# xbpeng/DeepMimic

Measured on NVIDIA H100. Metric: env-steps/sec (30 Hz policy steps; humanoid3d_spinkick, 4096 envs/GPU), higher is better.
Workload: dtype f32

## Files before the change

deepmimic_b200/capi.py:

```python
import ctypes as C
import os

import numpy as np

_REPO = os.path.dirname(os.path.dirname(os.path.abspath(__file__)))
_LIB_PATH = os.environ.get("DM_LIB", os.path.join(_REPO, "deepmimic_b200", "libdeepmimic_b200.so"))
_lib = None


class DmDims(C.Structure):
    _fields_ = [(n, C.c_int) for n in ("num_envs", "num_joints", "pose_dim", "num_dofs", "state_size", "goal_size", "action_size", "snapshot_size",
                                        "updates_per_action", "num_update_substeps")] + [("motion_duration", C.c_double), ("amp_obs_size", C.c_int)]


_fp = C.POINTER(C.c_float)


class DmMlpGatedWeights(C.Structure):
    _fields_ = ([(n, C.c_int) for n in ("in_dim", "goal_dim", "h0", "h1", "out_dim", "gate_common", "gate_hidden")]
                + [(n, _fp) for n in ("w0", "b0", "w1", "b1", "w2", "b2", "gc_w", "gc_b")]
                + [(n, _fp * 2) for n in ("gh_w", "gh_b", "gs_w", "gs_b", "gb_w", "gb_b")]
                + [(n, _fp) for n in ("s_mean", "s_std", "g_mean", "g_std", "a_mean", "a_std")] + [("s_clip", C.c_float), ("g_clip", C.c_float)])


# ... 6 lines not shown
                + [(n, C.c_void_p) for n in ("norm_actions", "old_logp", "adv", "logstd", "bound_min", "bound_max")]
                + [("ratio_clip", C.c_float), ("ratio", C.c_void_p), ("norm_targets", C.c_void_p)]
                + [(n, C.c_float) for n in ("stepsize", "momentum", "weight_decay")] + [("stats", C.c_void_p)])


class DmLearnDiscBatch(C.Structure):
    _fields_ = ([(n, C.c_void_p) for n in ("agent", "expert", "agent_idx", "expert_idx")] + [("rows", C.c_int), ("in_mean", C.c_void_p),
                ("in_istd", C.c_void_p), ("in_clip", C.c_float)]
                + [(n, C.c_float) for n in ("stepsize", "momentum", "weight_decay", "logit_reg_weight", "grad_penalty_weight")] + [("stats", C.c_void_p)])


class DmLearnGatedNet(C.Structure):
    _fields_ = [(n, C.c_void_p * 10) for n in ("w", "b", "acc_w", "acc_b")]


class DmLearnGatedBatch(C.Structure):
    _anonymous_ = ("batch",)
    _fields_ = [("batch", DmLearnBatch), ("goals", C.c_void_p), ("g_mean", C.c_void_p), ("g_istd", C.c_void_p), ("g_clip", C.c_float)]


DM_STATE_OFFSET, DM_STATE_SCALE, DM_ACTION_OFFSET, DM_ACTION_SCALE, DM_ACTION_BOUND_MIN, DM_ACTION_BOUND_MAX, DM_STATE_NORM_GROUPS = range(7)

EXPORTS = ["dm_create", "dm_load_host", "dm_plan_launch", "dm_get_model_info", "dm_get_link_table", "dm_destroy", "dm_last_error", "dm_get_dims", "dm_get_static", "dm_get_scene_name", "dm_stream", "dm_sync", "dm_set_mode", "dm_set_sample_count", "dm_get_time_limits", "dm_reset", "dm_set_action",
           "dm_update", "dm_record_state", "dm_record_goal", "dm_goal_host", "dm_reset_clips", "dm_record_amp_obs_expert_clips", "dm_get_clip_table", "dm_get_task_state", "dm_set_task_state", "dm_get_task_params", "dm_calc_reward", "dm_calc_reward_imitate", "dm_record_amp_obs_agent", "dm_record_amp_obs_expert", "dm_amp_obs_host", "dm_sample_amp_obs_expert", "dm_expert_sample_count", "dm_observe", "dm_get_flags", "dm_step_host", "dm_step_host_reset", "dm_set_time_limits", "dm_exchange_create", "dm_exchange_connect", "dm_exchange_publish", "dm_exchange_acquire", "dm_exchange_release", "dm_exchange_status", "dm_exchange_destroy", "dm_set_timing", "dm_step_host_timing", "dm_get_snapshot",
           "dm_set_snapshot", "dm_get_counters", "dm_get_section_profile", "dm_mlp_create", "dm_mlp_forward", "dm_mlp_create_gated", "dm_mlp_forward_gated",
           "dm_mlp_forward_style_reward", "dm_mlp_launches", "dm_mlp_destroy", "dm_td_lambda_returns", "dm_mlp_set_weights_device", "dm_learn_create",
           "dm_mlp_set_normalizers_device", "dm_learn_set_weights", "dm_learn_step", "dm_learn_disc_step", "dm_learn_destroy",
           "dm_learn_create_gated", "dm_learn_set_gated_weights", "dm_learn_gated_step", "dm_mlp_set_gated_weights_device", "dm_mlp_set_gated_normalizers_device"]


def lib():
    global _lib
    if _lib is None:
        if not os.path.exists(_LIB_PATH):
            raise RuntimeError("deepmimic_b200: %s is missing -- run `python -c 'import __graft_entry__ as g; g.build()'`. "
                               "There is no CPU fallback." % _LIB_PATH)
        L = C.CDLL(_LIB_PATH)
        vp, dp, fp, ip = C.c_void_p, C.POINTER(C.c_double), C.c_void_p, C.c_void_p
        L.dm_create.restype = vp
        L.dm_create.argtypes = [C.c_char_p, C.c_int, C.POINTER(C.c_char_p), C.c_int, C.c_int, C.c_uint64, C.c_uint64]
        L.dm_destroy.argtypes = [vp]
        L.dm_load_host.restype = vp
        L.dm_load_host.argtypes = [C.c_char_p, C.c_int, C.POINTER(C.c_char_p)]
        L.dm_get_model_info.argtypes = [vp, C.c_int, C.POINTER(C.c_int)]
        L.dm_plan_launch.argtypes = [vp, C.c_int, C.c_int, C.c_int, C.POINTER(C.c_int)]
        L.dm_get_link_table.argtypes = [vp, dp]
        L.dm_last_error.restype = C.c_char_p
        L.dm_get_dims.argtypes = [vp, C.POINTER(DmDims)]
        L.dm_get_static.argtypes = [vp, C.c_int, dp]
        L.dm_get_scene_name.argtypes = [vp, C.c_char_p, C.c_int]
        L.dm_stream.restype = vp
        L.dm_stream.argtypes = [vp]
        L.dm_sync.argtypes = [vp]
        L.dm_set_mode.argtypes = [vp, C.c_int]
        L.dm_set_sample_count.argtypes = [vp, C.c_longlong]
        L.dm_get_time_limits.argtypes = [vp, dp]
        L.dm_reset.argtypes = [vp, C.c_int, dp, dp, dp]
        L.dm_set_action.argtypes = [vp, fp]
        L.dm_update.argtypes = [vp, C.c_double, C.c_int]
        L.dm_record_state.argtypes = [vp, fp]
        L.dm_record_goal.argtypes = [vp, fp]
        L.dm_calc_reward.argtypes = [vp, fp]
        L.dm_calc_reward_imitate.argtypes = [vp, fp]
        L.dm_goal_host.argtypes = [vp, fp]
        L.dm_reset_clips.argtypes = [vp, C.c_int, C.POINTER(C.c_int), dp, dp, dp]
        L.dm_record_amp_obs_expert_clips.argtypes = [vp, C.POINTER(C.c_int), dp, fp]
        L.dm_get_clip_table.argtypes = [vp, C.POINTER(C.c_int), dp, dp]
        L.dm_get_task_state.argtypes = [vp, C.c_int, dp]
        L.dm_set_task_state.argtypes = [vp, C.c_int, dp]
        L.dm_get_task_params.argtypes = [vp, dp, C.POINTER(C.c_uint64)]
        L.dm_record_amp_obs_agent.argtypes = [vp, fp]
        L.dm_record_amp_obs_expert.argtypes = [vp, dp, fp]
        L.dm_amp_obs_host.argtypes = [vp, C.c_int, dp, fp]
        L.dm_sample_amp_obs_expert.argtypes = [vp, C.c_int, vp, vp, vp]
        L.dm_expert_sample_count.argtypes = [vp, C.POINTER(C.c_uint64), C.POINTER(C.c_uint64)]
        L.dm_observe.argtypes = [vp, fp, fp]
        L.dm_get_flags.argtypes = [vp, ip]
        L.dm_step_host.argtypes = [vp, fp, C.c_double, C.c_int, fp, fp, ip]
        L.dm_step_host_reset.argtypes = [vp, fp, C.c_double, C.c_int, fp, fp, ip, C.c_int]
        L.dm_set_time_limits.argtypes = [vp, C.c_double, C.c_double]
        L.dm_exchange_create.argtypes = [vp, C.c_int, C.c_int, C.c_void_p]
        L.dm_exchange_connect.argtypes = [vp, C.c_void_p]
# ... 48 lines not shown


def _dptr(a):
    return a.ctypes.data_as(C.POINTER(C.c_double)) if a is not None else None


def _call(fn, *args, stream=None):
    if getattr(lib(), fn)(*args, C.c_void_p(stream) if stream else None) != 0:
        raise RuntimeError("%s: %s" % (fn, lib().dm_last_error().decode()))


def td_lambda_returns(rewards, values, end_values, done, terminate, discount, td_lambda, val_fail, val_succ, returns, advantages, stream=None):
    T, N = rewards.shape
    for name, x, dt in (("rewards", rewards, "float32"), ("values", values, "float32"), ("end_values", end_values, "float32"), ("returns", returns, "float32"),
                        ("advantages", advantages, "float32"), ("done", done, ("bool", "uint8")), ("terminate", terminate, "int32")):
        if tuple(x.shape) != (T, N) or not x.is_contiguous() or not x.is_cuda or str(x.dtype).replace("torch.", "") not in (dt if isinstance(dt, tuple) else (dt,)):
            raise ValueError("td_lambda_returns: %s must be a contiguous %s CUDA tensor [%d, %d]" % (name, dt, T, N))
    ptr = lambda t: C.c_void_p(t.data_ptr())
    _call("dm_td_lambda_returns", ptr(rewards), ptr(values), ptr(end_values), ptr(done), ptr(terminate), T, N, float(discount), float(td_lambda),
          float(val_fail), float(val_succ), ptr(returns), ptr(advantages), stream=stream)
    return returns, advantages


class BatchedCore:

    def __init__(self, args, num_envs, asset_root, device=0, seed=0, global_env_offset=0):
        L = lib()
        enc = [a.encode() for a in args]
        arr = (C.c_char_p * len(enc))(*enc)
        self.h = L.dm_create(asset_root.encode(), len(enc), arr, num_envs, device, seed, global_env_offset)
        if not self.h:
            raise RuntimeError("dm_create failed: %s" % L.dm_last_error().decode())
        self.h = C.c_void_p(self.h)
        d = DmDims()
        L.dm_get_dims(self.h, C.byref(d))
        self.dims = d
        self.num_envs = d.num_envs

    def _chk(self, rc):
        if rc != 0:
            raise RuntimeError("deepmimic_b200: %s" % lib().dm_last_error().decode())

    def close(self):
        if self.h:
            lib().dm_destroy(self.h)
            self.h = None
# ... 16 lines not shown
        return buf.value.decode()

    def reset(self, force_all=True, kin_time=None, max_time=None, rot_theta=None, clip=None):
        f = lambda a: None if a is None else np.ascontiguousarray(a, dtype=np.float64)
        kt, mt, th = f(kin_time), f(max_time), f(rot_theta)
        if clip is None:
            self._chk(lib().dm_reset(self.h, 1 if force_all else 0, _dptr(kt), _dptr(mt), _dptr(th)))
        else:
            c = np.ascontiguousarray(clip, dtype=np.int32)
            self._chk(lib().dm_reset_clips(self.h, 1 if force_all else 0, c.ctypes.data_as(C.POINTER(C.c_int)), _dptr(kt), _dptr(mt), _dptr(th)))

    def clip_table(self):
        n = C.c_int(0)
        lib().dm_get_clip_table(self.h, C.byref(n), None, None)
        dur, cdf = np.zeros(n.value), np.zeros(n.value)
        lib().dm_get_clip_table(self.h, C.byref(n), _dptr(dur), _dptr(cdf))
        return dur, cdf

    def set_action(self, actions):
        self._chk(lib().dm_set_action(self.h, C.c_void_p(actions.data_ptr())))

    def update(self, dt, n_updates=1):
        self._chk(lib().dm_update(self.h, dt, n_updates))

    def observe(self, state=None, reward=None):
        self._chk(lib().dm_observe(self.h, C.c_void_p(state.data_ptr()) if state is not None else None,
                                   C.c_void_p(reward.data_ptr()) if reward is not None else None))

    def reward_imitate(self, out):
        self._chk(lib().dm_calc_reward_imitate(self.h, C.c_void_p(out.data_ptr())))

    def record_goal(self, out):
        self._chk(lib().dm_record_goal(self.h, C.c_void_p(out.data_ptr())))

    def goal_host(self):
        out = np.zeros((self.num_envs, self.dims.goal_size), dtype=np.float32)
        self._chk(lib().dm_goal_host(self.h, C.c_void_p(out.ctypes.data)))
        return out

    def task_state(self, env):
        out = np.zeros(24, dtype=np.float64)
        self._chk(lib().dm_get_task_state(self.h, env, _dptr(out)))
        return out

    def set_task_state(self, env, block):
        b = np.ascontiguousarray(block, dtype=np.float64)
# ... 414 lines not shown
```

deepmimic_b200/csrc/capi.cu:

```cuda
#include <cuda_runtime.h>

#include <algorithm>
#include <map>
#include <mutex>
#include <cmath>
#include <cstddef>
#include <cstdio>
#include <cstdlib>
#include <numeric>
#include <cstring>
#include <ctime>
#include <utility>
#include <memory>
#include <string>
#include <vector>

#include "../../include/deepmimic_b200.h"
#include "host/assets.hpp"
#include "kernels/dm_model.cuh"

namespace dmk {
__global__ void dm_flags_kernel(DevState st, int32_t* out, int num_real_envs) {
    int e = blockIdx.x * blockDim.x + threadIdx.x;
    if (e >= num_real_envs) return;
// ... 43 lines not shown
        cudaError_t e_ = (call);                                                                              \
        if (e_ != cudaSuccess) { g_err = std::string(#call) + ": " + cudaGetErrorString(e_); return fail(); } \
    } while (0)

struct dm_handle {
    dmh::SceneAssets sa;
    dmk::DevModel hm;
    dmk::DevModel* d_model = nullptr;
    dmk::DevState st{};
    double* d_frame_times = nullptr;
    float* d_frames = nullptr;
    float* d_frame_vel = nullptr;
    double* d_inj[3] = {nullptr, nullptr, nullptr};
    int32_t* d_flags4 = nullptr;
    float *d_amp = nullptr, *p_amp = nullptr;
    float *d_goal = nullptr, *p_goal = nullptr;
    dmk::ClipTable ctab{};
    dmk::ClipTable* d_ctab = nullptr; int* d_clip_inj = nullptr;
    int total_frames = 0;
    float *d_act = nullptr, *d_obs = nullptr, *d_rew = nullptr;
    float *p_act = nullptr, *p_obs = nullptr, *p_rew = nullptr; int32_t* p_flags = nullptr;
    cudaStream_t stream = nullptr;
    int device = 0, num_envs = 0, padded_envs = 0, W = 32, tiles = 2, maxrows = 36, smem_bytes = 0, mode = 0;
    dmk::StepLayout lay{};
    uint64_t seed = 0, env_offset = 0;
    int64_t launches = 0;
    uint64_t amp_calls = 0;
    uint64_t expert_samples = 0;
    std::vector<double> st_off, st_scale, act_off, act_scale, act_min, act_max, st_groups;
    std::vector<std::pair<const void*, bool>> pin_cache;
    int x_rank = 0, x_world = 0;
    char* x_base = nullptr;
    char* x_peer[8] = {nullptr, nullptr, nullptr, nullptr, nullptr, nullptr, nullptr, nullptr};
    size_t x_data_off = 0, x_parity_bytes = 0;
    bool timing = false;
    cudaEvent_t tev[5] = {nullptr, nullptr, nullptr, nullptr, nullptr};
    double host_ms[3] = {0, 0, 0};
    std::vector<void*> dev_bufs, pinned_bufs;
};

namespace {

int fail() { std::fprintf(stderr, "[deepmimic_b200] %s\n", g_err.c_str()); return 1; }

using dmh::Quat; using dmh::V3;
inline void put3(float* o, const V3& v, double s = 1.0) { o[0] = static_cast<float>(s * v.x); o[1] = static_cast<float>(s * v.y); o[2] = static_cast<float>(s * v.z); }
// ... 202 lines not shown
}

bool task_scene(const dm_handle* h) { return h->hm.task_kind != dmk::kTaskNone; }
int goal_size(const dmk::DevModel& M) { return M.task_kind == dmk::kTaskNone ? 0 : (M.task_kind >= dmk::kTaskHeadingGetup ? 4 : 3); }
int tile_index(const dm_handle* h) { return h->W == 32 ? 1 : 0; }
int policy_grid(const dm_handle* h) { return h->padded_envs / (dmk::kPolicyBlock / h->W); }

int launched(dm_handle* h) {
    DM_CUDA(cudaGetLastError());
    h->launches++;
    return 0;
}

int launch_step(dm_handle* h, double dt, int n_updates) {
    const dmk::StepKernel kern = dmk::kStepKernels[tile_index(h)][task_scene(h)];
    static std::mutex mu;
    static std::map<std::pair<int, const void*>, int> configured;
    {
        std::lock_guard<std::mutex> lock(mu);
        int& have = configured[{h->device, reinterpret_cast<const void*>(kern)}];
        if (h->smem_bytes > have) {
            DM_CUDA(cudaFuncSetAttribute(kern, cudaFuncAttributeMaxDynamicSharedMemorySize, h->smem_bytes));
            DM_CUDA(cudaFuncSetAttribute(kern, cudaFuncAttributePreferredSharedMemoryCarveout, 100));
            have = h->smem_bytes;
        }
    }
    kern<<<h->padded_envs / h->tiles, h->tiles * h->W, h->smem_bytes, h->stream>>>(h->d_model, h->st, h->d_frame_times, h->d_frames, dt, n_updates,
                                                                                   h->sa.cfg.num_sim_substeps, h->lay);
    return launched(h);
}
int launch_observe_fan(dm_handle* h, const dmk::ObsFan& fan) {
    const dmk::ObserveKernel kern = dmk::kObserveKernels[tile_index(h)][task_scene(h)];
    const size_t smem = static_cast<size_t>(dmk::kPolicyBlock / h->W) * h->hm.state_size * sizeof(float);
    kern<<<policy_grid(h), dmk::kPolicyBlock, smem, h->stream>>>(h->d_model, h->st, h->d_frame_times, h->d_frames, h->d_frame_vel, fan, h->num_envs);
    return launched(h);
}
int launch_observe(dm_handle* h, float* d_state, float* d_reward) {
    dmk::ObsFan fan{};
    fan.n = 1; fan.obs[0] = d_state; fan.rew[0] = d_reward; fan.done[0] = nullptr;
    return launch_observe_fan(h, fan);
}
int launch_reset(dm_handle* h, int force, const double* kt, const double* mt, const double* th, const int* clip) {
    const dmk::ResetKernel kern = dmk::kResetKernels[tile_index(h)][task_scene(h)];
    kern<<<policy_grid(h), dmk::kPolicyBlock, 0, h->stream>>>(h->d_model, h->st, h->d_frame_times, h->d_frames, h->d_frame_vel, force, kt, mt, th, h->seed,
                                                              h->env_offset, h->mode, clip);
    return launched(h);
}
int launch_amp(dm_handle* h, float* d_out, int expert, const double* d_times, const int* d_clips) {
// ... 197 lines not shown
    h->ctab = dmk::ClipTable{};
    h->ctab.num_clips = static_cast<int>(h->sa.clips.size());
    for (size_t c = 0; c < h->sa.clips.size(); ++c) {
        const dmh::MotionClip& mc = h->sa.clips[c];
        dmk::ClipInfo& ci = h->ctab.info[c];
        ci.dur = mc.duration(); ci.frame_off = h->total_frames; ci.num_frames = mc.num_frames; ci.loop = mc.loop ? 1 : 0;
        const double* fb = mc.frame(0); const double* fe = mc.frame(mc.num_frames - 1);
        ci.cycle_delta[0] = static_cast<float>(fe[0] - fb[0]); ci.cycle_delta[1] = 0.f; ci.cycle_delta[2] = static_cast<float>(fe[2] - fb[2]);
        h->ctab.cdf[c] = h->sa.clip_cdf[c];
        ci.is_getup = std::find(h->sa.cfg.getup_motion_ids.begin(), h->sa.cfg.getup_motion_ids.end(), static_cast<int>(c)) != h->sa.cfg.getup_motion_ids.end() ? 1 : 0;
        h->total_frames += mc.num_frames;
    }
    const size_t TF = static_cast<size_t>(h->total_frames);
    DM_CUDA(cudaStreamCreateWithFlags(&h->stream, cudaStreamNonBlocking));
    if (alloc_buffer(h, &h->d_model, 1) || alloc_buffer(h, &h->st.sim, N * ss) || alloc_buffer(h, &h->st.time, N * dmk::kTimeDoubles, kZeroed) ||
        alloc_buffer(h, &h->st.flags, N * dmk::kFlagInts, kZeroed) || alloc_buffer(h, &h->st.manifold, N * M.nl * dmk::kManifoldFloats, kZeroed) ||
        alloc_buffer(h, &h->d_frame_times, TF) || alloc_buffer(h, &h->d_frames, TF * M.pose_dim) || alloc_buffer(h, &h->d_frame_vel, TF * M.pose_dim) ||
        alloc_buffer(h, &h->d_flags4, N * 4) || alloc_buffer(h, &h->d_amp, N * M.amp_obs_size) || alloc_buffer(h, &h->p_amp, N * M.amp_obs_size, kPinned) ||
        alloc_buffer(h, &h->st.hist, N * 2 * M.pose_dim, kZeroed) || alloc_buffer(h, &h->d_act, N * std::max(1, M.action_size)) ||
        alloc_buffer(h, &h->d_obs, N * M.state_size) || alloc_buffer(h, &h->d_rew, N) || alloc_buffer(h, &h->p_act, N * std::max(1, M.action_size), kPinned) ||
        alloc_buffer(h, &h->p_obs, N * M.state_size, kPinned) || alloc_buffer(h, &h->p_rew, N, kPinned) || alloc_buffer(h, &h->p_flags, N * 4, kPinned))
        return 1;
    for (auto& p : h->d_inj) if (alloc_buffer(h, &p, N)) return 1;
#ifdef DM_PROFILE
    if (alloc_buffer(h, &h->st.prof, static_cast<size_t>(h->padded_envs / h->tiles) * (h->tiles * h->W / 32) * dmk::kProfCounters, kZeroed)) return 1;
#endif
    h->st.num_envs = h->padded_envs; h->st.num_real = h->num_envs;
    if (task_scene(h)) {
        if (alloc_buffer(h, &h->st.task, N * dmk::kTaskDoubles, kZeroed) || alloc_buffer(h, &h->st.taskx, N * dmk::kTaskExtDoubles, kZeroed) ||
            alloc_buffer(h, &h->d_goal, N * 4) || alloc_buffer(h, &h->p_goal, N * 4, kPinned) || alloc_buffer(h, &h->st.clip, N, kZeroed) ||
            alloc_buffer(h, &h->d_clip_inj, N) || alloc_buffer(h, &h->d_ctab, 1))
            return 1;
        DM_CUDA(cudaMemcpy(h->d_ctab, &h->ctab, sizeof(dmk::ClipTable), cudaMemcpyHostToDevice));
    }
    h->st.ctab = h->d_ctab;
    std::vector<float> frames(TF * M.pose_dim), fvel(frames.size());
    std::vector<double> ftimes(TF);
    for (size_t c = 0; c < h->sa.clips.size(); ++c) {
        const dmh::MotionClip& mc = h->sa.clips[c];
        const std::vector<double> fv = build_frame_vel(h->sa.character, mc);
        const size_t off = static_cast<size_t>(h->ctab.info[c].frame_off);
        std::copy(mc.frame_times.begin(), mc.frame_times.end(), ftimes.begin() + off);
        for (size_t i = 0; i < mc.frames.size(); ++i) { frames[off * M.pose_dim + i] = static_cast<float>(mc.frames[i]); fvel[off * M.pose_dim + i] = static_cast<float>(fv[i]); }
    }
    DM_CUDA(cudaMemcpy(h->d_model, &h->hm, sizeof(dmk::DevModel), cudaMemcpyHostToDevice));
    DM_CUDA(cudaMemcpy(h->d_frame_times, ftimes.data(), sizeof(double) * TF, cudaMemcpyHostToDevice));
// ... 109 lines not shown
    for (int k = 0; k < 3; ++k) if (src[k] && stage_envs(h, src[k], h->d_inj[k])) return 1;
    if (h_clip && stage_envs(h, h_clip, h->d_clip_inj)) return 1;
    if (launch_reset(h, force_all, kt ? h->d_inj[0] : nullptr, mt ? h->d_inj[1] : nullptr, th ? h->d_inj[2] : nullptr, h_clip ? h->d_clip_inj : nullptr)) return 1;
    if (!task_scene(h)) return 0;
    dmk::dm_task_reset_kernel<<<(h->padded_envs + 127) / 128, 128, 0, h->stream>>>(h->d_model, h->st, h->padded_envs);
    return launched(h);
}
int dm_reset(dm_handle* h, int force_all, const double* kt, const double* mt, const double* th) { return dm_reset_clips(h, force_all, nullptr, kt, mt, th); }
int dm_get_clip_table(dm_handle* h, int* num_clips, double* h_dur, double* h_cdf) {
    const int n = static_cast<int>(h->sa.clips.size());
    if (num_clips) *num_clips = n;
    for (int c = 0; c < n; ++c) { if (h_dur) h_dur[c] = h->sa.clips[c].duration(); if (h_cdf) h_cdf[c] = h->sa.clip_cdf[c]; }
    return 0;
}
int dm_set_action(dm_handle* h, const float* d_actions) {
    DM_DEVICE(h);
    const int total = h->num_envs * h->hm.nl;
    dmk::dm_set_action_kernel<<<(total + 127) / 128, 128, 0, h->stream>>>(h->d_model, h->st, d_actions, h->num_envs);
    return launched(h);
}
int dm_update(dm_handle* h, double dt, int n_updates) {
    DM_DEVICE(h);
    return launch_step(h, dt, n_updates);
}
static int launch_task_observe(dm_handle* h, float* d_goal, float* d_reward) {
    dmk::dm_task_observe_kernel<<<(h->num_envs + 127) / 128, 128, 0, h->stream>>>(h->d_model, h->st, d_goal, d_reward, h->num_envs);
    return launched(h);
}
int dm_observe(dm_handle* h, float* d_state, float* d_reward) {
    DM_DEVICE(h);
    const bool task = task_scene(h);
    float* d_imitate_reward = task ? nullptr : d_reward;
    if ((d_state != nullptr || d_imitate_reward != nullptr) && launch_observe(h, d_state, d_imitate_reward)) return 1;
    if (task && d_reward != nullptr) return launch_task_observe(h, nullptr, d_reward);
    return 0;
}
int dm_record_state(dm_handle* h, float* d_out) { return dm_observe(h, d_out, nullptr); }
int dm_calc_reward_imitate(dm_handle* h, float* d_out) {
    DM_DEVICE(h);
    return launch_observe(h, nullptr, d_out);
}
int dm_record_goal(dm_handle* h, float* d_out) {
    if (!task_scene(h)) return 0;
    DM_DEVICE(h);
    return launch_task_observe(h, d_out, nullptr);
}
// ... 361 lines not shown
```

deepmimic_b200/csrc/kernels/dm_model.cuh:

```cuda
#pragma once
#include <cstdint>

#include "dm_math.cuh"

#include "dm_task.cuh"
#include "dm_task_ext.cuh"

namespace dmk {

constexpr int kMaxLinks = 32;
constexpr int kMaxDofs = 96;
constexpr int kMaxChain = 24;
constexpr int kMaxChildren = 4;
constexpr int kStepMaxThreads = 448;
constexpr int kStepRegs = 128;
constexpr int kManifoldFloats = 48;
constexpr int kProfCounters = 18;

enum DevJointType { kJRevolute = 0, kJSpherical = 1, kJFixed = 2 };
enum DevShape { kSBox = 1, kSCapsule = 2, kSSphere = 3 };

struct DevLink {
    int parent, jtype, ndof, dof0;
    int level, nchild, child[kMaxChildren];
// ... 70 lines not shown
    while (lo < hi) { const int mid = (lo + hi) >> 1; if (t.cdf[mid] <= u) lo = mid + 1; else hi = mid; }
    return lo < t.num_clips ? lo : t.num_clips - 1;
}

__host__ __device__ inline int sim_stride(int nl) { return 16 + 12 * nl; }
constexpr int kTimeDoubles = 16;
enum TimeSlot { kTKin = 0, kTCtrl = 1, kTInitOff = 2, kTPrevAct = 3, kTTimer = 4, kTTimerMax = 5, kTOrigin = 6, kTOriginRot = 9 };
constexpr int kFlagInts = 8;
enum FlagSlot { kFNeedAction = 0, kFDone = 1, kFTerminate = 2, kFValid = 3, kFFallen = 4, kFRowOverflow = 5, kFUpdates = 6 };

struct DevState {
    float* sim;
    double* time;
    int* flags;
    float* manifold;
    float* hist;
    unsigned int* prof;
    double* task;
    double* taskx;
    int* clip;
    const ClipTable* ctab;
    int num_envs;
    int num_real;
};

constexpr int kMaxFan = 8;
struct ObsFan {
    int n;
    float* obs[kMaxFan];
    float* rew[kMaxFan];
    float* done[kMaxFan];
};

__host__ __device__ constexpr int dm_step_y_stride(int W) { return W == 16 ? 32 : 52; }

struct StepLayout {
    int nl, n, chain_len, maxrows, maxpts;
    int oU, oR, oA, oW, oV, oY, oLam, oRhs, oInv, oRl, oPp, oPi, oPr, oQ, oG, oZ;
    int env_floats, hot_floats;
};

constexpr int kPolicyBlock = 64;
using StepKernel = void (*)(const DevModel*, DevState, const double*, const float*, double, int, int, StepLayout);
using ObserveKernel = void (*)(const DevModel*, DevState, const double*, const float*, const float*, ObsFan, int);
using ResetKernel = void (*)(const DevModel*, DevState, const double*, const float*, const float*, int, const double*, const double*, const double*,
                             unsigned long long, unsigned long long, int, const int*);
using AmpObsKernel = void (*)(const DevModel*, DevState, const double*, const float*, const float*, float*, int, const double*, int, const int*);
extern const StepKernel kStepKernels[2][2];
extern const ObserveKernel kObserveKernels[2][2];
extern const ResetKernel kResetKernels[2][2];
extern const AmpObsKernel kAmpObsKernels[2][2];
using AmpExpertKernel = void (*)(const DevModel*, DevState, const double*, const float*, const float*, float*, int, unsigned long long, unsigned long long,
                                 int*, double*);
extern const AmpExpertKernel kAmpExpertKernels[2][2];
__global__ void dm_set_action_kernel(const DevModel*, DevState, const float*, int);
__global__ void dm_task_reset_kernel(const DevModel*, DevState, int);
__global__ void dm_task_observe_kernel(const DevModel*, DevState, float*, float*, int);
int dm_step_layout(int nl, int n, int chain_len, int maxrows, int W, StepLayout* L);
int dm_step_smem_bytes(const StepLayout& L, int tiles);

}
```

deepmimic_b200/csrc/kernels/dm_step.cu:

```cuda
#include "dm_model.cuh"
#include <type_traits>

namespace dmk {

namespace {

template <int W>
struct Tl {
    static __device__ __forceinline__ float shfl(float v, int src) { return __shfl_sync(0xffffffffu, v, src, W); }
    static __device__ __forceinline__ int shfli(int v, int src) { return __shfl_sync(0xffffffffu, v, src, W); }
    static __device__ __forceinline__ V3 shfl3(V3 v, int src) { return mk3(shfl(v.x, src), shfl(v.y, src), shfl(v.z, src)); }
    static __device__ __forceinline__ S6 shfl6(S6 v, int src) { return mks(shfl3(v.a, src), shfl3(v.l, src)); }
};
__device__ __forceinline__ void ld12(const float* p, float* o) {
    const float4 a = reinterpret_cast<const float4*>(p)[0], b = reinterpret_cast<const float4*>(p)[1], c_ = reinterpret_cast<const float4*>(p)[2];
    o[0] = a.x; o[1] = a.y; o[2] = a.z; o[3] = a.w; o[4] = b.x; o[5] = b.y; o[6] = b.z; o[7] = b.w; o[8] = c_.x; o[9] = c_.y; o[10] = c_.z; o[11] = c_.w;
}
__device__ __forceinline__ void st12(float* p, const float* o) {
    reinterpret_cast<float4*>(p)[0] = make_float4(o[0], o[1], o[2], o[3]); reinterpret_cast<float4*>(p)[1] = make_float4(o[4], o[5], o[6], o[7]);
    reinterpret_cast<float4*>(p)[2] = make_float4(o[8], o[9], o[10], o[11]);
}
__device__ __forceinline__ float rcp_fast(float x) { float r; asm("rcp.approx.ftz.f32 %0, %1;" : "=f"(r) : "f"(x)); return r; }
__device__ __forceinline__ int wmax(int v) {
#pragma unroll
// ... 943 lines not shown
    if (c.jtype == kJSpherical) jww = jvx * S0 + jvy * S1 + jvz * S2; else if (c.jtype == kJRevolute) jww = jvx * S0;
    S6 vel = mks(mk3(0, 0, 0), mk3(0, 0, 0));
    if (c.lane == 0) { const V3 bo = mk3(sB[7], sB[8], sB[9]); vel = mks(bo + jww, mk3(sB[10], sB[11], sB[12]) + cross(bo, cw)); }
#pragma unroll 1
    for (int lv = 1; lv <= c.maxlevel; ++lv) {
        const S6 pv = T::shfl6(vel, c.plane);
        if (c.level == lv) vel = mks(pv.a + jww, pv.l + cross(pv.a, cw));
    }
    if (c.act && want) {
        float* v = sV + c.lane * 12;
        v[0] = vel.a.x; v[1] = vel.a.y; v[2] = vel.a.z; v[3] = vel.l.x; v[4] = vel.l.y; v[5] = vel.l.z;
    }
    __syncwarp();
}

template <int W, bool TASK>
__global__ void __launch_bounds__(kStepMaxThreads, 1) dm_step_kernel(const DevModel* __restrict__ gm, DevState st, const double* __restrict__ frame_times,
                                                                       const float* __restrict__ frames, double dt, int n_updates, int sim_substeps, StepLayout LY) {
    using T = Tl<W>;
    extern __shared__ __align__(16) float sm[];
    const int tiles = blockDim.x / W;
    const int tile = threadIdx.x / W;
    const int lane = threadIdx.x % W;
    const int env = blockIdx.x * tiles + tile;
    const DevModel& M = *gm;
    const int nl = LY.nl, CL = LY.chain_len;
    const bool act = lane < nl;
    const int li = act ? lane : nl - 1;

    float* LK = sm + kHdrFloats;
    unsigned char* CD = reinterpret_cast<unsigned char*>(LK + nl * kLkFloats);
    unsigned char* CH = CD + nl * nl;
    int* LYS = reinterpret_cast<int*>(sm + kHLayout);
    for (int j = threadIdx.x; j < nl; j += blockDim.x) {
        const DevLink& K = M.link[j];
        float* q = LK + j * kLkFloats;
        const int p = K.parent;
        for (int k = 0; k < 3; ++k) { q[kLC + k] = K.evec[k] + (p >= 0 ? M.link[p].dvec[k] : 0.f); q[kLD + k] = K.dvec[k]; q[kLAx + k] = K.axis[k]; }
        q[kLM] = K.mass;
        auto lumped = [&](int c_) { const DevLink& C_ = M.link[c_]; return C_.ndof == 0 && C_.nchild == 0 && C_.parent >= 0 && M.link[C_.parent].ndof > 0; };
        const bool isroot = p < 0, self_lumped = lumped(j);
        {
            float cm = 0.f, mdx = 0.f, mdy = 0.f, mdz = 0.f, wD[6] = {0, 0, 0, 0, 0, 0}, wB[6] = {0, 0, 0, 0, 0, 0};
            auto add_part = [&](float m_, V3 r, const float* iD, const float* iB) {
                const float rr = dot(r, r);
                const float sh[6] = {m_ * (rr - r.x * r.x), -m_ * r.x * r.y, -m_ * r.x * r.z, m_ * (rr - r.y * r.y), -m_ * r.y * r.z, m_ * (rr - r.z * r.z)};
                for (int k = 0; k < 6; ++k) { wD[k] += iD[k] + sh[k]; wB[k] += iB[k] + sh[k]; }
// ... 89 lines not shown
    int f_over = fl[kFRowOverflow], f_updates = fl[kFUpdates];
    __syncwarp();

    const float h = static_cast<float>(dt) / static_cast<float>(sim_substeps);
    const float fdt = static_cast<float>(dt);
    const float gx = M.gravity[0], gy = M.gravity[1], gz = M.gravity[2];
    const float scale = M.scale, mu = M.friction;

    float tau0 = 0.f, tau1 = 0.f, tau2 = 0.f;
    bool in_contact_tol = false;

#ifdef DM_PROFILE
    unsigned int* PRF = reinterpret_cast<unsigned int*>(sm + LY.hot_floats + tiles * LY.env_floats) + (threadIdx.x / 32) * kProfCounters;
    if ((threadIdx.x & 31) == 0) for (int k = 0; k < kProfCounters; ++k) PRF[k] = 0u;
    unsigned int prf_t = static_cast<unsigned int>(clock64());
#define PROF(sec) do { if ((threadIdx.x & 31) == 0) { unsigned int t_ = static_cast<unsigned int>(clock64()); PRF[sec] += t_ - prf_t; prf_t = t_; } } while (0)
    unsigned int* PRFP = PRF;
#else
#define PROF(sec) do { } while (0)
    unsigned int* PRFP = nullptr;
#endif
    bool need_kin = true, pending_flags = false;
    int mcnt = 4;
    const int stages_per_upd = sim_substeps + 1;
    const int total_stages = n_updates * stages_per_upd;
#pragma unroll 1
    for (int stage = 0; stage <= total_stages; ++stage) {
        if ((stage % stages_per_upd) != 0 && act && alive && mcnt > 0) {
            const float* mp_ = mani + li * kManifoldFloats;
            asm volatile("prefetch.global.L1 [%0];" ::"l"(mp_));
            asm volatile("prefetch.global.L1 [%0];" ::"l"(mp_ + 32));
        }
        if (need_kin) { need_kin = false; kin_pass<W>(jp, jv); }
        PROF(0);
        if (pending_flags) {
            pending_flags = false;
            need_action = cbits & 1;
            const unsigned fb = __ballot_sync(0xffffffffu, act && fall_contact && in_contact_tol);
            const unsigned fseg = (W == 32) ? fb : ((fb >> (threadIdx.x & 16)) & 0xffffu);
            const int fallen = (fseg != 0 && M.enable_contact_fall) ? 1 : 0;
            const float* v = sV + li * 12;
            const V3 wa = mk3(v[0], v[1], v[2]);
            const V3 vw = (mk3(v[3], v[4], v[5]) + cross(wa, mk3(v[6], v[7], v[8]))) * (1.0f / scale);
            float mx = fmaxf(fmaxf(fmaxf(fabsf(vw.x), fabsf(vw.y)), fabsf(vw.z)), fmaxf(fmaxf(fabsf(wa.x), fabsf(wa.y)), fabsf(wa.z)));
            const unsigned eb = __ballot_sync(0xffffffffu, act && mx > 100.f);
            const unsigned eseg = (W == 32) ? eb : ((eb >> (threadIdx.x & 16)) & 0xffffu);
// ... 34 lines not shown
                        if (kind == kTaskHeadingGetup) {
                            tkx[kXHeadY] = B.head_y;
                            if (getup_update(M.taskx, tkx, dt, M.test_mode != 0, fallen != 0)) fe = 0;
                        }
                    }
                }
                task_fail = T::shfli(tf, 0);
                fallen_eff = T::shfli(fe, 0);
            }
            if (alive) {
                int term = (M.enable_fall_end && fallen_eff) ? 1 : 0;
                if (!term && (cbits & 4)) term = 1;
                if (TASK && !term && task_fail) term = task_fail;
                f_updates++;
                const bool end = (cbits & 2) || term;
                if (end || stage == total_stages) {
                    if (lane == 0) {
                        reinterpret_cast<float4*>(sim)[0] = make_float4(sB[0], sB[1], sB[2], 0.f);
                        reinterpret_cast<float4*>(sim)[1] = make_float4(sB[3], sB[4], sB[5], sB[6]);
                        reinterpret_cast<float4*>(sim)[2] = make_float4(sB[7], sB[8], sB[9], 0.f);
                        reinterpret_cast<float4*>(sim)[3] = make_float4(sB[10], sB[11], sB[12], 0.f);
                        fl[kFNeedAction] = need_action; fl[kFDone] = end ? 1 : 0; fl[kFTerminate] = term; fl[kFValid] = (eseg == 0) ? 1 : 0; fl[kFFallen] = fallen_eff;
                        fl[kFRowOverflow] = f_over; fl[kFUpdates] = f_updates;
                    }
                    if (act) {
                        reinterpret_cast<float4*>(sim + 16)[lane] = jp;
                        reinterpret_cast<float4*>(sim + 16 + 4 * nl)[lane] = jv;
                    }
                }
                if (end) alive = false;
            }
        }
        PROF(1);
        if (stage == total_stages) break;
        if (__syncthreads_and(!alive)) break;
        PROF(2);
        if (__ballot_sync(0xffffffffu, alive) == 0u) {
            if ((stage % stages_per_upd) != 0)
                for (int k = 0; k < kSubstepBarriers; ++k) __syncthreads();
            continue;
        }
        const int ph = stage % stages_per_upd;
        if (ph == 0) {
            int cb = 0;
            if constexpr (TASK) {
                if (__ballot_sync(0xffffffffu, alive && need_action) != 0u) {
// ... 70 lines not shown
            bool hit = false;
            if (ndof >= 1) { const float v = jv.x + h * qdd.x; jv.x = cl100(v); hit |= fabsf(v) > 100.f; }
            if (ndof == 3) { const float v1 = jv.y + h * qdd.y, v2 = jv.z + h * qdd.z; jv.y = cl100(v1); jv.z = cl100(v2); hit |= fabsf(v1) > 100.f || fabsf(v2) > 100.f; }
            if (lane == 0) for (int k = 0; k < 6; ++k) hit |= fabsf(sB[7 + k]) >= 100.f;
            const unsigned hb = __ballot_sync(0xffffffffu, hit);
            if (hb != 0u) {
                const unsigned hseg = (W == 32) ? hb : ((hb >> (threadIdx.x & 16)) & 0xffffu);
                vel_pass<W>(jv.x, jv.y, jv.z, hseg != 0u);
            }
        }
        PROF(ph == 1 ? 16 : 17);
        __syncthreads();
        PROF(2);
        int lim_dir = 0; float lim_pen = 0.f;
        if (act && has_limit && alive) {
            float p0 = jp.x - LKo[kLLo], p1 = LKo[kLHi] - jp.x;
            if (!(p0 > 0.f)) { lim_dir = 1; lim_pen = p0; }
            else if (!(p1 > 0.f)) { lim_dir = -1; lim_pen = p1; }
        }
        const unsigned lbal = __ballot_sync(0xffffffffu, lim_dir != 0);
        const unsigned lseg = (W == 32) ? lbal : ((lbal >> (threadIdx.x & 16)) & 0xffffu);
        int NL = __popc(lseg);
        const unsigned anyrow = __ballot_sync(0xffffffffu, NL + P > 0);
        if (anyrow != 0) {
            {
                const int lidx = __popc(lseg & ((1u << lane) - 1u));
                if (NL > 8) { NL = 8; f_over = 1; }
                if (lim_dir != 0 && lidx < 8) { sQ[lidx] = __int_as_float(lane); sQ[8 + lidx] = (lim_dir == -1) ? -1.f : 1.f; sQ[16 + lidx] = lim_pen; sQ[24 + lidx] = jv.x; }
            }
            if (NL + 3 * P > LY.maxrows) { P = (LY.maxrows - NL) / 3; f_over = 1; }
            const int NR = NL + 3 * P;
            __syncwarp();
            PROF(5);
#ifdef DM_PROFILE
            { const int nrm = wmax(NR); if ((threadIdx.x & 31) == 0) { PRF[13] += nrm; PRF[14] += 1; if (nrm > W) PRF[15] += 1; } }
#endif
            solve_rows<W>(NL, P, mani, alive ? 1 : 0, PRFP);
            PROF(10);
            const float3 dq = dv_pass<W>();
            if (NR > 0) {
                if (ndof >= 1) jv.x = cl100(jv.x + dq.x);
                if (ndof == 3) { jv.y = cl100(jv.y + dq.y); jv.z = cl100(jv.z + dq.z); }
            }
            PROF(11);
        }
        __syncthreads();
        PROF(2);
        if (lane == 0) {
            sB[0] += h * sB[10]; sB[1] += h * sB[11]; sB[2] += h * sB[12];
            const Q4 q = quat_integrate3(mk3(sB[7], sB[8], sB[9]), mkq(sB[3], sB[4], sB[5], sB[6]), true, h);
            sB[3] = q.x; sB[4] = q.y; sB[5] = q.z; sB[6] = q.w;
        }
        if (jtype == kJRevolute) jp.x += h * jv.x;
        else if (jtype == kJSpherical) { Q4 q = quat_integrate3(mk3(jv.x, jv.y, jv.z), mkq(jp.x, jp.y, jp.z, jp.w), false, h); jp = make_float4(q.x, q.y, q.z, q.w); }
        __syncwarp();
        need_kin = true;
        if (ph == sim_substeps) pending_flags = true;
        PROF(12);
    }
#ifdef DM_PROFILE
    __syncwarp();
    if ((threadIdx.x & 31) == 0 && st.prof) { unsigned int* o = st.prof + (blockIdx.x * (blockDim.x / 32) + threadIdx.x / 32) * kProfCounters; for (int k = 0; k < kProfCounters; ++k) o[k] = PRF[k]; }
#endif
}

const StepKernel kStepKernels[2][2] = {{dm_step_kernel<16, false>, dm_step_kernel<16, true>}, {dm_step_kernel<32, false>, dm_step_kernel<32, true>}};

}
```

include/deepmimic_b200.h:

```cpp
#ifndef DEEPMIMIC_B200_H_
#define DEEPMIMIC_B200_H_
#include <stddef.h>
#include <stdint.h>
#ifdef __cplusplus
extern "C" {
#endif

typedef struct dm_handle dm_handle;

typedef struct dm_dims {
    int num_envs;
    int num_joints;
    int pose_dim;
    int num_dofs;
    int state_size;
    int goal_size;
    int action_size;
    int snapshot_size;
    int updates_per_action;
    int num_update_substeps;
    double motion_duration;
    int amp_obs_size;
} dm_dims;

// ... 6 lines not shown
dm_handle* dm_load_host(const char* asset_root, int argc, const char** argv);
int dm_plan_launch(dm_handle* h, int num_envs, int smem_bytes_per_block, int num_sms, int* out9);
enum dm_model_info_kind {
    DM_INFO_PARENTS = 0, DM_INFO_JOINT_TYPES = 1 , DM_INFO_DOF_OFFSETS = 2, DM_INFO_POSE_OFFSETS = 3,
    DM_INFO_FALL_BODIES = 4, DM_INFO_END_EFFECTORS = 5, DM_INFO_LAYOUT = 6
};
int dm_get_model_info(dm_handle* h, int kind, int* out);
int dm_get_link_table(dm_handle* h, double* h_out);
void dm_destroy(dm_handle* h);
const char* dm_last_error(void);
int dm_get_dims(dm_handle* h, dm_dims* out);
int dm_get_scene_name(dm_handle* h, char* h_out, int capacity);
int dm_get_static(dm_handle* h, int kind, double* h_out);
void* dm_stream(dm_handle* h);
int dm_sync(dm_handle* h);
int dm_set_mode(dm_handle* h, int mode);
int dm_set_sample_count(dm_handle* h, long long count);
int dm_set_time_limits(dm_handle* h, double t_min, double t_max);
int dm_get_time_limits(dm_handle* h, double* h_out3);

int dm_reset(dm_handle* h, int force_all, const double* h_kin_time, const double* h_max_time, const double* h_rot_theta);
int dm_set_action(dm_handle* h, const float* d_actions);
int dm_update(dm_handle* h, double dt, int n_updates);
int dm_record_state(dm_handle* h, float* d_out);
int dm_record_goal(dm_handle* h, float* d_out);
int dm_goal_host(dm_handle* h, float* h_out);
int dm_reset_clips(dm_handle* h, int force_all, const int* h_clip, const double* h_kin_time, const double* h_max_time, const double* h_rot_theta);
int dm_record_amp_obs_expert_clips(dm_handle* h, const int* h_clip, const double* h_kin_time, float* d_out);
int dm_get_clip_table(dm_handle* h, int* num_clips, double* h_dur, double* h_cdf);
int dm_get_task_state(dm_handle* h, int env, double* h_out16);
int dm_set_task_state(dm_handle* h, int env, const double* h_in16);
int dm_get_task_params(dm_handle* h, double* h_out48, unsigned long long* h_stream2);
int dm_calc_reward(dm_handle* h, float* d_out);
int dm_calc_reward_imitate(dm_handle* h, float* d_out);
int dm_record_amp_obs_agent(dm_handle* h, float* d_out);
int dm_record_amp_obs_expert(dm_handle* h, const double* h_kin_time, float* d_out);
int dm_amp_obs_host(dm_handle* h, int expert, const double* h_kin_time, float* h_out);
int dm_sample_amp_obs_expert(dm_handle* h, int rows, float* d_out, int* d_clip_out, double* d_time_out);
int dm_expert_sample_count(dm_handle* h, const unsigned long long* h_set, unsigned long long* h_get);
int dm_observe(dm_handle* h, float* d_state, float* d_reward);
int dm_get_flags(dm_handle* h, int32_t* d_flags);

int dm_step_host(dm_handle* h, const float* h_actions, double dt, int n_updates, float* h_state, float* h_reward, int32_t* h_flags);
int dm_step_host_reset(dm_handle* h, const float* h_actions, double dt, int n_updates, float* h_state, float* h_reward, int32_t* h_flags, int reset_done);
int dm_set_timing(dm_handle* h, int on);
int dm_step_host_timing(dm_handle* h, double* h_out8);
// ... 96 lines not shown
```

Measured before the change: 2.444 million.

## Reorder environments by contact-row load to balance warps in step kernel

Records each env's contact-row count from the last substep and, before every step launch, runs a single-block counting-sort kernel that buckets envs by load. It assigns them to block/warp slots in a serpentine pattern, so envs with similar load share a warp and heavy envs are spread across blocks. This targets warp divergence and tail imbalance in the W=16 physics kernel. It adds an extra single-block launch per update and an indirection on env indexing, which can reduce memory coalescing.

```diff
diff --git a/deepmimic_b200/capi.py b/deepmimic_b200/capi.py
--- a/deepmimic_b200/capi.py
+++ b/deepmimic_b200/capi.py
@@ -52,7 +52,7 @@
 DM_STATE_OFFSET, DM_STATE_SCALE, DM_ACTION_OFFSET, DM_ACTION_SCALE, DM_ACTION_BOUND_MIN, DM_ACTION_BOUND_MAX, DM_STATE_NORM_GROUPS = range(7)
 
 EXPORTS = ["dm_create", "dm_load_host", "dm_plan_launch", "dm_get_model_info", "dm_get_link_table", "dm_destroy", "dm_last_error", "dm_get_dims", "dm_get_static", "dm_get_scene_name", "dm_stream", "dm_sync", "dm_set_mode", "dm_set_sample_count", "dm_get_time_limits", "dm_reset", "dm_set_action",
-           "dm_update", "dm_record_state", "dm_record_goal", "dm_goal_host", "dm_reset_clips", "dm_record_amp_obs_expert_clips", "dm_get_clip_table", "dm_get_task_state", "dm_set_task_state", "dm_get_task_params", "dm_calc_reward", "dm_calc_reward_imitate", "dm_record_amp_obs_agent", "dm_record_amp_obs_expert", "dm_amp_obs_host", "dm_sample_amp_obs_expert", "dm_expert_sample_count", "dm_observe", "dm_get_flags", "dm_step_host", "dm_step_host_reset", "dm_set_time_limits", "dm_exchange_create", "dm_exchange_connect", "dm_exchange_publish", "dm_exchange_acquire", "dm_exchange_release", "dm_exchange_status", "dm_exchange_destroy", "dm_set_timing", "dm_step_host_timing", "dm_get_snapshot",
+           "dm_update", "dm_set_env_order", "dm_plan_env_order", "dm_get_env_order", "dm_record_state", "dm_record_goal", "dm_goal_host", "dm_reset_clips", "dm_record_amp_obs_expert_clips", "dm_get_clip_table", "dm_get_task_state", "dm_set_task_state", "dm_get_task_params", "dm_calc_reward", "dm_calc_reward_imitate", "dm_record_amp_obs_agent", "dm_record_amp_obs_expert", "dm_amp_obs_host", "dm_sample_amp_obs_expert", "dm_expert_sample_count", "dm_observe", "dm_get_flags", "dm_step_host", "dm_step_host_reset", "dm_set_time_limits", "dm_exchange_create", "dm_exchange_connect", "dm_exchange_publish", "dm_exchange_acquire", "dm_exchange_release", "dm_exchange_status", "dm_exchange_destroy", "dm_set_timing", "dm_step_host_timing", "dm_get_snapshot",
            "dm_set_snapshot", "dm_get_counters", "dm_get_section_profile", "dm_mlp_create", "dm_mlp_forward", "dm_mlp_create_gated", "dm_mlp_forward_gated",
            "dm_mlp_forward_style_reward", "dm_mlp_launches", "dm_mlp_destroy", "dm_td_lambda_returns", "dm_mlp_set_weights_device", "dm_learn_create",
            "dm_mlp_set_normalizers_device", "dm_learn_set_weights", "dm_learn_step", "dm_learn_disc_step", "dm_learn_destroy",
@@ -88,6 +88,9 @@
         L.dm_reset.argtypes = [vp, C.c_int, dp, dp, dp]
         L.dm_set_action.argtypes = [vp, fp]
         L.dm_update.argtypes = [vp, C.c_double, C.c_int]
+        L.dm_set_env_order.argtypes = [vp, C.c_int]
+        L.dm_plan_env_order.argtypes = [C.POINTER(C.c_int), C.c_int, C.c_int, C.c_int, C.POINTER(C.c_int)]
+        L.dm_get_env_order.argtypes = [vp, C.POINTER(C.c_int), C.POINTER(C.c_int), C.POINTER(C.c_int)]
         L.dm_record_state.argtypes = [vp, fp]
         L.dm_record_goal.argtypes = [vp, fp]
         L.dm_calc_reward.argtypes = [vp, fp]
@@ -182,6 +185,15 @@
     return returns, advantages
 
 
+def plan_env_order(keys, tiles, tile_width):
+    k = np.ascontiguousarray(keys, dtype=np.int32)
+    out = np.zeros(len(k), dtype=np.int32)
+    ip = C.POINTER(C.c_int)
+    if lib().dm_plan_env_order(k.ctypes.data_as(ip), len(k), int(tiles), int(tile_width), out.ctypes.data_as(ip)) != 0:
+        raise RuntimeError(lib().dm_last_error().decode())
+    return out
+
+
 class BatchedCore:
 
     def __init__(self, args, num_envs, asset_root, device=0, seed=0, global_env_offset=0):
@@ -244,6 +256,17 @@
 
     def update(self, dt, n_updates=1):
         self._chk(lib().dm_update(self.h, dt, n_updates))
+
+    def set_env_order(self, on):
+        self._chk(lib().dm_set_env_order(self.h, 1 if on else 0))
+
+    def env_order(self):
+        ip = C.POINTER(C.c_int)
+        plan = np.zeros(3, dtype=np.int32)
+        self._chk(lib().dm_get_env_order(self.h, plan.ctypes.data_as(ip), None, None))
+        keys, order = np.zeros(plan[0], dtype=np.int32), np.zeros(plan[0], dtype=np.int32)
+        self._chk(lib().dm_get_env_order(self.h, plan.ctypes.data_as(ip), keys.ctypes.data_as(ip), order.ctypes.data_as(ip)))
+        return keys, order, int(plan[1]), int(plan[2])
 
     def observe(self, state=None, reward=None):
         self._chk(lib().dm_observe(self.h, C.c_void_p(state.data_ptr()) if state is not None else None,
diff --git a/deepmimic_b200/csrc/capi.cu b/deepmimic_b200/csrc/capi.cu
--- a/deepmimic_b200/csrc/capi.cu
+++ b/deepmimic_b200/csrc/capi.cu
@@ -89,6 +89,7 @@
     float *p_act = nullptr, *p_obs = nullptr, *p_rew = nullptr; int32_t* p_flags = nullptr;
     cudaStream_t stream = nullptr;
     int device = 0, num_envs = 0, padded_envs = 0, W = 32, tiles = 2, maxrows = 36, smem_bytes = 0, mode = 0;
+    int* d_order = nullptr;
     dmk::StepLayout lay{};
     uint64_t seed = 0, env_offset = 0;
     int64_t launches = 0;
@@ -337,8 +338,13 @@
         if (h->smem_bytes > have) {
             DM_CUDA(cudaFuncSetAttribute(kern, cudaFuncAttributeMaxDynamicSharedMemorySize, h->smem_bytes));
             DM_CUDA(cudaFuncSetAttribute(kern, cudaFuncAttributePreferredSharedMemoryCarveout, 100));
+            DM_CUDA(cudaFuncSetAttribute(dmk::dm_env_order_kernel, cudaFuncAttributePreferredSharedMemoryCarveout, 100));
             have = h->smem_bytes;
         }
+    }
+    if (h->st.order) {
+        dmk::dm_env_order_kernel<<<1, dmk::kEnvOrderThreads, 0, h->stream>>>(h->st.load, h->padded_envs, h->tiles, h->W, h->d_order);
+        if (launched(h)) return 1;
     }
     kern<<<h->padded_envs / h->tiles, h->tiles * h->W, h->smem_bytes, h->stream>>>(h->d_model, h->st, h->d_frame_times, h->d_frames, dt, n_updates,
                                                                                    h->sa.cfg.num_sim_substeps, h->lay);
@@ -582,6 +588,15 @@
         alloc_buffer(h, &h->p_obs, N * M.state_size, kPinned) || alloc_buffer(h, &h->p_rew, N, kPinned) || alloc_buffer(h, &h->p_flags, N * 4, kPinned))
         return 1;
     for (auto& p : h->d_inj) if (alloc_buffer(h, &p, N)) return 1;
+    if (alloc_buffer(h, &h->st.load, N) || alloc_buffer(h, &h->d_order, N)) return 1;
+    {
+        std::vector<int> load(N, 0), ident(N);
+        std::fill(load.begin() + h->num_envs, load.end(), dmk::kLoadPadding);
+        std::iota(ident.begin(), ident.end(), 0);
+        DM_CUDA(cudaMemcpy(h->st.load, load.data(), N * sizeof(int), cudaMemcpyHostToDevice));
+        DM_CUDA(cudaMemcpy(h->d_order, ident.data(), N * sizeof(int), cudaMemcpyHostToDevice));
+    }
+    h->st.order = (h->W == 16) ? h->d_order : nullptr;
 #ifdef DM_PROFILE
     if (alloc_buffer(h, &h->st.prof, static_cast<size_t>(h->padded_envs / h->tiles) * (h->tiles * h->W / 32) * dmk::kProfCounters, kZeroed)) return 1;
 #endif
@@ -737,6 +752,31 @@
 int dm_update(dm_handle* h, double dt, int n_updates) {
     DM_DEVICE(h);
     return launch_step(h, dt, n_updates);
+}
+int dm_set_env_order(dm_handle* h, int on) {
+    DM_DEVICE(h);
+    h->st.order = (on && h->W == 16) ? h->d_order : nullptr;
+    return 0;
+}
+int dm_plan_env_order(const int* keys, int n_padded, int tiles, int W, int* order) {
+    if (!keys || !order || (W != 16 && W != 32) || tiles <= 0 || tiles % (32 / W) != 0 || n_padded <= 0 || n_padded % tiles != 0) {
+        g_err = "dm_plan_env_order: bad arguments";
+        return fail();
+    }
+    std::vector<int> sorted(n_padded);
+    std::iota(sorted.begin(), sorted.end(), 0);
+    std::stable_sort(sorted.begin(), sorted.end(), [&](int a, int b) { return dmk::env_load_bucket(keys[a]) < dmk::env_load_bucket(keys[b]); });
+    for (int r = 0; r < n_padded; ++r) order[dmk::env_order_slot(r, n_padded, tiles, W)] = sorted[r];
+    return 0;
+}
+int dm_get_env_order(dm_handle* h, int* h_plan3, int* h_keys, int* h_order) {
+    DM_DEVICE(h);
+    if (h_plan3) { h_plan3[0] = h->padded_envs; h_plan3[1] = h->tiles; h_plan3[2] = h->W; }
+    DM_CUDA(cudaStreamSynchronize(h->stream));
+    if (h_keys) DM_CUDA(cudaMemcpy(h_keys, h->st.load, sizeof(int) * h->padded_envs, cudaMemcpyDeviceToHost));
+    if (h_order && h->st.order) DM_CUDA(cudaMemcpy(h_order, h->st.order, sizeof(int) * h->padded_envs, cudaMemcpyDeviceToHost));
+    else if (h_order) std::iota(h_order, h_order + h->padded_envs, 0);
+    return 0;
 }
 static int launch_task_observe(dm_handle* h, float* d_goal, float* d_reward) {
     dmk::dm_task_observe_kernel<<<(h->num_envs + 127) / 128, 128, 0, h->stream>>>(h->d_model, h->st, d_goal, d_reward, h->num_envs);
diff --git a/deepmimic_b200/csrc/kernels/dm_model.cuh b/deepmimic_b200/csrc/kernels/dm_model.cuh
--- a/deepmimic_b200/csrc/kernels/dm_model.cuh
+++ b/deepmimic_b200/csrc/kernels/dm_model.cuh
@@ -116,7 +116,19 @@
     const ClipTable* ctab;
     int num_envs;
     int num_real;
+    int* load;
+    const int* order;
 };
+
+constexpr int kLoadPadding = -1;
+constexpr int kLoadBuckets = 64;
+__host__ __device__ inline int env_load_bucket(int key) { const int b = kLoadBuckets - 2 - key; return b < 0 ? 0 : (b >= kLoadBuckets ? kLoadBuckets - 1 : b); }
+__host__ __device__ inline int env_order_slot(int r, int n_padded, int tiles, int W) {
+    const int per_warp = 32 / W, blocks = n_padded / tiles, warps = tiles / per_warp;
+    const int g = r / per_warp, round = g / blocks, j = g % blocks;
+    const int b = (round & 1) ? blocks - 1 - j : j;
+    return (b * warps + round) * per_warp + r % per_warp;
+}
 
 constexpr int kMaxFan = 8;
 struct ObsFan {
@@ -147,6 +159,8 @@
 using AmpExpertKernel = void (*)(const DevModel*, DevState, const double*, const float*, const float*, float*, int, unsigned long long, unsigned long long,
                                  int*, double*);
 extern const AmpExpertKernel kAmpExpertKernels[2][2];
+constexpr int kEnvOrderThreads = 1024;
+__global__ void dm_env_order_kernel(const int* load, int n_padded, int tiles, int W, int* order);
 __global__ void dm_set_action_kernel(const DevModel*, DevState, const float*, int);
 __global__ void dm_task_reset_kernel(const DevModel*, DevState, int);
 __global__ void dm_task_observe_kernel(const DevModel*, DevState, float*, float*, int);
diff --git a/deepmimic_b200/csrc/kernels/dm_step.cu b/deepmimic_b200/csrc/kernels/dm_step.cu
--- a/deepmimic_b200/csrc/kernels/dm_step.cu
+++ b/deepmimic_b200/csrc/kernels/dm_step.cu
@@ -989,7 +989,8 @@
     const int tiles = blockDim.x / W;
     const int tile = threadIdx.x / W;
     const int lane = threadIdx.x % W;
-    const int env = blockIdx.x * tiles + tile;
+    const int slot = blockIdx.x * tiles + tile;
+    const int env = (W == 16 && st.order) ? st.order[slot] : slot;
     const DevModel& M = *gm;
     const int nl = LY.nl, CL = LY.chain_len;
     const bool act = lane < nl;
@@ -1125,6 +1126,7 @@
 #endif
     bool need_kin = true, pending_flags = false;
     int mcnt = 4;
+    int last_nr = 0;
     const int stages_per_upd = sim_substeps + 1;
     const int total_stages = n_updates * stages_per_upd;
 #pragma unroll 1
@@ -1205,6 +1207,7 @@
                         reinterpret_cast<float4*>(sim)[3] = make_float4(sB[10], sB[11], sB[12], 0.f);
                         fl[kFNeedAction] = need_action; fl[kFDone] = end ? 1 : 0; fl[kFTerminate] = term; fl[kFValid] = (eseg == 0) ? 1 : 0; fl[kFFallen] = fallen_eff;
                         fl[kFRowOverflow] = f_over; fl[kFUpdates] = f_updates;
+                        if (W == 16) st.load[env] = last_nr;
                     }
                     if (act) {
                         reinterpret_cast<float4*>(sim + 16)[lane] = jp;
@@ -1321,6 +1324,7 @@
         const unsigned lseg = (W == 32) ? lbal : ((lbal >> (threadIdx.x & 16)) & 0xffffu);
         int NL = __popc(lseg);
         const unsigned anyrow = __ballot_sync(0xffffffffu, NL + P > 0);
+        last_nr = 0;
         if (anyrow != 0) {
             {
                 const int lidx = __popc(lseg & ((1u << lane) - 1u));
@@ -1329,6 +1333,7 @@
             }
             if (NL + 3 * P > LY.maxrows) { P = (LY.maxrows - NL) / 3; f_over = 1; }
             const int NR = NL + 3 * P;
+            last_nr = NR;
             __syncwarp();
             PROF(5);
 #ifdef DM_PROFILE
@@ -1365,4 +1370,71 @@
 
 const StepKernel kStepKernels[2][2] = {{dm_step_kernel<16, false>, dm_step_kernel<16, true>}, {dm_step_kernel<32, false>, dm_step_kernel<32, true>}};
 
-}
+constexpr int kEnvOrderItems = 4;
+__global__ void __launch_bounds__(kEnvOrderThreads) dm_env_order_kernel(const int* __restrict__ load, int n_padded, int tiles, int W, int* __restrict__ order) {
+    constexpr int kWarps = kEnvOrderThreads / 32, kCells = kEnvOrderItems * kWarps, kChunk = kEnvOrderItems * kEnvOrderThreads;
+    constexpr int kParts = kEnvOrderThreads / kLoadBuckets, kPer = kCells / kParts;
+    static_assert(kParts <= 32 && 32 % kParts == 0 && kCells % kParts == 0, "the scan of a bucket's cells runs inside one warp");
+    __shared__ int base[kLoadBuckets];
+    __shared__ int cnt[kLoadBuckets][kCells + 1];
+    const int t = threadIdx.x, warp = t / 32, lane = t % 32;
+    const unsigned lt = (1u << lane) - 1u;
+    int b[kEnvOrderItems];
+    auto load_chunk = [&](int c0) {
+#pragma unroll
+        for (int i = 0; i < kEnvOrderItems; ++i) { const int e = c0 + i * kEnvOrderThreads + t; b[i] = (e < n_padded) ? env_load_bucket(load[e]) : kLoadBuckets; }
+    };
+    auto count = [&](int bk) {
+        const unsigned peers = __match_any_sync(0xffffffffu, bk);
+        if (bk < kLoadBuckets && (peers & lt) == 0) atomicAdd(&base[bk], __popc(peers));
+    };
+    load_chunk(0);
+    if (t < kLoadBuckets) base[t] = 0;
+    __syncthreads();
+#pragma unroll
+    for (int i = 0; i < kEnvOrderItems; ++i) count(b[i]);
+    for (int e = kChunk + t; e < n_padded + t; e += kEnvOrderThreads) count((e < n_padded) ? env_load_bucket(load[e]) : kLoadBuckets);
+    __syncthreads();
+    if (warp == 0) {
+        const int c0 = base[2 * lane], c1 = base[2 * lane + 1];
+        int incl = c0 + c1;
+#pragma unroll
+        for (int o = 1; o < 32; o <<= 1) { const int v = __shfl_up_sync(0xffffffffu, incl, o); if (lane >= o) incl += v; }
+        base[2 * lane] = incl - c0 - c1; base[2 * lane + 1] = incl - c1;
+    }
+    const int sb = t / kParts, part = t % kParts;
+    for (int c0 = 0; c0 < n_padded; c0 += kChunk) {
+        if (c0 > 0) load_chunk(c0);
+        for (int k = t; k < kLoadBuckets * (kCells + 1); k += kEnvOrderThreads) (&cnt[0][0])[k] = 0;
+        __syncthreads();
+        int below[kEnvOrderItems];
+#pragma unroll
+        for (int i = 0; i < kEnvOrderItems; ++i) {
+            const unsigned peers = __match_any_sync(0xffffffffu, b[i]);
+            below[i] = __popc(peers & lt);
+            if (b[i] < kLoadBuckets && below[i] == 0) cnt[b[i]][i * kWarps + warp] = __popc(peers);
+        }
+        __syncthreads();
+        {
+            int v[kPer], s = 0;
+#pragma unroll
+            for (int k = 0; k < kPer; ++k) { v[k] = cnt[sb][part * kPer + k]; s += v[k]; }
+            int incl = s;
+#pragma unroll
+            for (int o = 1; o < kParts; o <<= 1) { const int u = __shfl_up_sync(0xffffffffu, incl, o, kParts); if (part >= o) incl += u; }
+            const int first = base[sb];
+            int r = first + incl - s;
+#pragma unroll
+            for (int k = 0; k < kPer; ++k) { cnt[sb][part * kPer + k] = r; r += v[k]; }
+            __syncwarp();
+            if (part == kParts - 1) base[sb] = first + incl;
+        }
+        __syncthreads();
+#pragma unroll
+        for (int i = 0; i < kEnvOrderItems; ++i)
+            if (b[i] < kLoadBuckets) order[env_order_slot(cnt[b[i]][i * kWarps + warp] + below[i], n_padded, tiles, W)] = c0 + i * kEnvOrderThreads + t;
+        __syncthreads();
+    }
+}
+
+}
diff --git a/include/deepmimic_b200.h b/include/deepmimic_b200.h
--- a/include/deepmimic_b200.h
+++ b/include/deepmimic_b200.h
@@ -52,6 +52,9 @@
 int dm_reset(dm_handle* h, int force_all, const double* h_kin_time, const double* h_max_time, const double* h_rot_theta);
 int dm_set_action(dm_handle* h, const float* d_actions);
 int dm_update(dm_handle* h, double dt, int n_updates);
+int dm_set_env_order(dm_handle* h, int on);
+int dm_plan_env_order(const int* keys, int n_padded, int tiles, int W, int* order);
+int dm_get_env_order(dm_handle* h, int* h_plan3, int* h_keys, int* h_order);
 int dm_record_state(dm_handle* h, float* d_out);
 int dm_record_goal(dm_handle* h, float* d_out);
 int dm_goal_host(dm_handle* h, float* h_out);
```

New measurement: 2.530 million (median of 6 runs). +3.5%, better.
